# dalek-cryptography/curve25519-dalek

Hardware: NVIDIA H100
Metric: Pippenger MSM points/sec (higher is better)
Workload: dtype exact integers: f64 limbs (radix 2^51, FP64 pipe) in the bucket kernel, u32 limbs (radix 2^25.5) elsewhere

## Files before the change

curve25519_dalek_b200/csrc/api.cu:

```cuda
#include <cstring>
#include <new>
#include <random>

#include "../../include/dalek_b200.h"
#include "engine.h"

extern "C" {

int dalek_b200_init(int device, dalek_b200_ctx **out)
{
    if (!out) return DALEK_E_INVALID_ARG;
    *out = nullptr;
    int count = 0;
    if (cudaGetDeviceCount(&count) != cudaSuccess || count <= 0 || device < 0 || device >= count) return DALEK_E_NO_DEVICE;
    cudaDeviceProp prop;
    if (cudaGetDeviceProperties(&prop, device) != cudaSuccess) return DALEK_E_NO_DEVICE;
    if (prop.major != 9 || prop.minor != 0) return DALEK_E_NO_DEVICE;
    if (cudaSetDevice(device) != cudaSuccess) return DALEK_E_CUDA;
    dalek_b200_ctx *ctx = new (std::nothrow) dalek_b200_ctx();
    if (!ctx) return DALEK_E_NOMEM;
    ctx->device = device;
    ctx->sm_count = prop.multiProcessorCount;
    try { std::random_device rd; for (int i = 0; i < 4; i++) ctx->hash_seed[i] ^= rd(); } catch (...) { }
    int prio_lo = 0, prio_hi = 0;
    cudaDeviceGetStreamPriorityRange(&prio_lo, &prio_hi);
    if (cudaStreamCreateWithPriority(&ctx->stream, cudaStreamNonBlocking, prio_hi) != cudaSuccess ||
        cudaStreamCreateWithPriority(&ctx->stream2, cudaStreamNonBlocking, prio_lo) != cudaSuccess ||
        cudaStreamCreateWithFlags(&ctx->stream_copy, cudaStreamNonBlocking) != cudaSuccess ||
        cudaStreamCreateWithPriority(&ctx->stream3, cudaStreamNonBlocking, prio_hi) != cudaSuccess ||
        cudaStreamCreateWithPriority(&ctx->stream_hash, cudaStreamNonBlocking, prio_hi) != cudaSuccess ||
        cudaEventCreate(&ctx->ev_a) != cudaSuccess || cudaEventCreate(&ctx->ev_b) != cudaSuccess ||
        cudaEventCreate(&ctx->ev_call0) != cudaSuccess || cudaEventCreate(&ctx->ev_call1) != cudaSuccess ||
        cudaEventCreateWithFlags(&ctx->ev_fork, cudaEventDisableTiming) != cudaSuccess ||
        cudaEventCreateWithFlags(&ctx->ev_join, cudaEventDisableTiming) != cudaSuccess ||
        cudaEventCreateWithFlags(&ctx->ev_join2, cudaEventDisableTiming) != cudaSuccess) {
        delete ctx;
        return DALEK_E_CUDA;
    }
    for (int i = 0; i < 8; i++)
        if (cudaEventCreateWithFlags(&ctx->ev_grp[i], cudaEventDisableTiming) != cudaSuccess ||
            cudaEventCreateWithFlags(&ctx->ev_hram[i], cudaEventDisableTiming) != cudaSuccess || cudaEventCreate(&ctx->ev_prep[i][0]) != cudaSuccess ||
            cudaEventCreate(&ctx->ev_prep[i][1]) != cudaSuccess) { delete ctx; return DALEK_E_CUDA; }
    *out = ctx;
    return DALEK_OK;
}

void dalek_b200_destroy(dalek_b200_ctx *ctx)
{
    if (!ctx) return;
    cudaSetDevice(ctx->device);
    cudaStreamSynchronize(ctx->stream);
    cudaStreamSynchronize(ctx->stream2);
    cudaStreamSynchronize(ctx->stream3);
    cudaStreamSynchronize(ctx->stream_hash);
    DevBuf *bufs[] = {&ctx->scalars, &ctx->points_in, &ctx->points, &ctx->digits, &ctx->counts, &ctx->offsets,
                      &ctx->sorted, &ctx->buckets, &ctx->red_a, &ctx->red_b, &ctx->red_c, &ctx->red_d, &ctx->key_pts,
                      &ctx->result, &ctx->flags, &ctx->misc0, &ctx->misc1, &ctx->misc2, &ctx->misc3,
                      &ctx->misc4, &ctx->misc5, &ctx->zs, &ctx->base_table, &ctx->ntasks, &ctx->task_off, &ctx->tasks, &ctx->task_sums, &ctx->msg_offs, &ctx->sum_desc, &ctx->sum_part, &ctx->key_table, &ctx->key_acc, &ctx->task_order, &ctx->sig_status, &ctx->misc6, &ctx->each_pow, &ctx->each_tab, &ctx->each_kstat, &ctx->comb_base_table};
    for (DevBuf *b : bufs) if (b->p) cudaFree(b->p);
    if (ctx->h_pinned) cudaFreeHost(ctx->h_pinned);
    cudaEventDestroy(ctx->ev_a); cudaEventDestroy(ctx->ev_b); cudaEventDestroy(ctx->ev_fork); cudaEventDestroy(ctx->ev_join);
    cudaEventDestroy(ctx->ev_join2); cudaEventDestroy(ctx->ev_call0); cudaEventDestroy(ctx->ev_call1);
    for (int i = 0; i < 8; i++) { cudaEventDestroy(ctx->ev_grp[i]); cudaEventDestroy(ctx->ev_hram[i]); cudaEventDestroy(ctx->ev_prep[i][0]); cudaEventDestroy(ctx->ev_prep[i][1]); }
    cudaStreamDestroy(ctx->stream_hash);
    cudaStreamDestroy(ctx->stream); cudaStreamDestroy(ctx->stream2); cudaStreamDestroy(ctx->stream_copy); cudaStreamDestroy(ctx->stream3);
    delete ctx;
}

const char *dalek_b200_last_error(const dalek_b200_ctx *ctx) { return ctx ? ctx->last_error.c_str() : "null context"; }

int dalek_b200_set_option(dalek_b200_ctx *ctx, const char *name, long value)
{
    if (!ctx || !name) return DALEK_E_INVALID_ARG;
    if (!strcmp(name, "window_bits")) { if (value != 0 && (value < 4 || value > 20)) return DALEK_E_INVALID_ARG; ctx->opt_window_bits = value; return 0; }
    if (!strcmp(name, "host_chunks")) { if (value < 1 || value > 8) return DALEK_E_INVALID_ARG; ctx->opt_host_chunks = value; return 0; }
    if (!strcmp(name, "decompress_f64")) { ctx->opt_decompress_f64 = value ? 1 : 0; return 0; }
    if (!strcmp(name, "trace")) { ctx->opt_trace = value ? 1 : 0; return 0; }
    if (!strcmp(name, "precomp_tables")) { ctx->opt_precomp_tables = value ? 1 : 0; return 0; }
    if (!strcmp(name, "double_base_comb")) { ctx->opt_double_base_comb = value ? 1 : 0; return 0; }
    if (!strcmp(name, "dedupe_keys")) { ctx->opt_dedupe_keys = value ? 1 : 0; return 0; }
    if (!strcmp(name, "verify_pieces")) { if (value < 1 || value > 8) return DALEK_E_INVALID_ARG; ctx->opt_verify_pieces = value; return 0; }
    if (!strcmp(name, "transcript_warp")) { ctx->opt_transcript_warp = value ? 1 : 0; return 0; }
    if (!strcmp(name, "transcript_blocks")) { ctx->opt_transcript_blocks = value ? 1 : 0; return 0; }
    if (!strcmp(name, "each_comb")) { if (value < 0 || value > 2) return DALEK_E_INVALID_ARG; ctx->opt_each_comb = value; return 0; }
    if (!strcmp(name, "small_straus")) { ctx->opt_small_straus = value ? 1 : 0; return 0; }
    if (!strcmp(name, "acc_tma")) { ctx->opt_acc_tma = value ? 1 : 0; return 0; }
    if (!strcmp(name, "field_f64")) { ctx->opt_field_f64 = value ? 1 : 0; return 0; }
    if (!strcmp(name, "verify_chunk")) { if (value < 0 || value > (1 << 20)) return DALEK_E_INVALID_ARG; ctx->opt_verify_chunk = value; return 0; }
    return DALEK_E_INVALID_ARG;
}

uint64_t dalek_b200_launch_count(const dalek_b200_ctx *ctx) { return ctx ? ctx->launches : 0; }

int dalek_b200_last_kernel_ms(const dalek_b200_ctx *ctx, float *ms, int *launches)
{
    if (!ctx) return DALEK_E_INVALID_ARG;
    if (ms) *ms = ctx->last_kernel_ms;
    if (launches) *launches = ctx->last_kernel_launches;
    return 0;
}

int dalek_b200_last_stage_ms(const dalek_b200_ctx *ctx, const char *stage, float *ms)
{
    if (!ctx || !stage || !ms) return DALEK_E_INVALID_ARG;
    if (!strcmp(stage, "bucket_accumulate")) { *ms = ctx->last_kernel_ms; return 0; }
    if (!strcmp(stage, "decompress_R")) { *ms = ctx->last_prep_ms; return 0; }
    return DALEK_E_INVALID_ARG;
}

int dalek_b200_last_call_ms(const dalek_b200_ctx *ctx, float *ms)
{
    if (!ctx || !ms) return DALEK_E_INVALID_ARG;
    *ms = ctx->last_call_ms;
    return 0;
}

}

static int run_msm(dalek_b200_ctx *ctx, const void *scalars, const void *points_in, bool on_device, int point_fmt, size_t n,
                   size_t n_window ,
                   ge_p3_raw *d_windows, MsmResult *d_result)
{
    int rc;
    const size_t pin = msm_point_bytes(point_fmt);
    cudaStream_t st = ctx->stream;
    const int c = msm_choose_window_bits(ctx, n_window);
    const bool straus = d_result && n == n_window && n < STRAUS_VT_THRESHOLD && ctx->opt_small_straus && ctx->opt_field_f64;
    const int kind = msm_prepared_kind(point_fmt, straus ? PK_PNIELS : PK_NIELS);
    const size_t psz = kind == PK_NIELS ? sizeof(ge_niels_packed) : sizeof(ge_pniels_packed);
    if ((rc = ws_reserve(ctx, ctx->points, std::max<size_t>(1, n) * psz))) return rc;
    if ((rc = ws_reserve(ctx, ctx->flags, 64))) return rc;
    CUDA_TRY(ctx, cudaMemsetAsync(ctx->flags.p, 0, 64, st));
    if (on_device) {
        if (straus) {
            if ((rc = msm_prepare_points(ctx, points_in, point_fmt, n, ctx->points.p, (int *)ctx->flags.p, kind))) return rc;
            if ((rc = straus_vartime_msm(ctx, (const uint32_t *)scalars, ctx->points.p, kind, n, d_result))) return rc;
        } else {
            CUDA_TRY(ctx, cudaEventRecord(ctx->ev_fork, st));
            CUDA_TRY(ctx, cudaStreamWaitEvent(ctx->stream2, ctx->ev_fork, 0));
            if ((rc = msm_prepare_points_on(ctx, ctx->stream2, points_in, point_fmt, n, ctx->points.p, (int *)ctx->flags.p))) return rc;
            CUDA_TRY(ctx, cudaEventRecord(ctx->ev_join, ctx->stream2));
            if ((rc = msm_accumulate_chunk(ctx, (const uint32_t *)scalars, (const ge_niels_packed *)ctx->points.p, n, c, true, 0, 0, ctx->ev_join))) return rc;
        }
    } else {
        if ((rc = ws_reserve(ctx, ctx->scalars, std::max<size_t>(1, n) * 32))) return rc;
        if ((rc = ws_reserve(ctx, ctx->points_in, std::max<size_t>(1, n) * pin))) return rc;
        int K = n >= (1u << 18) ? (int)std::min<long>(8, std::max<long>(1, ctx->opt_host_chunks)) : 1;
        CUDA_TRY(ctx, cudaEventRecord(ctx->ev_fork, st));
        CUDA_TRY(ctx, cudaStreamWaitEvent(ctx->stream_copy, ctx->ev_fork, 0));
        CUDA_TRY(ctx, cudaStreamWaitEvent(ctx->stream2, ctx->ev_fork, 0));
        for (int k = 0; k < K; k++) {
            const size_t i0 = n * k / K, i1 = n * (k + 1) / K, cnt = i1 - i0;
            char *ds = (char *)ctx->scalars.p + i0 * 32, *dp = (char *)ctx->points_in.p + i0 * pin;
            if (cnt) {
                CUDA_TRY(ctx, cudaMemcpyAsync(ds, (const char *)scalars + i0 * 32, cnt * 32, cudaMemcpyHostToDevice, ctx->stream_copy));
                CUDA_TRY(ctx, cudaMemcpyAsync(dp, (const char *)points_in + i0 * pin, cnt * pin, cudaMemcpyHostToDevice, ctx->stream_copy));
            }
            CUDA_TRY(ctx, cudaEventRecord(ctx->ev_grp[k], ctx->stream_copy));
            CUDA_TRY(ctx, cudaStreamWaitEvent(st, ctx->ev_grp[k], 0));
            char *dq = (char *)ctx->points.p + i0 * psz;
            if (straus) {
                if ((rc = msm_prepare_points(ctx, dp, point_fmt, cnt, dq, (int *)ctx->flags.p, kind))) return rc;
                if ((rc = straus_vartime_msm(ctx, (const uint32_t *)ds, dq, kind, cnt, d_result))) return rc;
            } else {
                CUDA_TRY(ctx, cudaStreamWaitEvent(ctx->stream2, ctx->ev_grp[k], 0));
                if ((rc = msm_prepare_points_on(ctx, ctx->stream2, dp, point_fmt, cnt, dq, (int *)ctx->flags.p))) return rc;
                CUDA_TRY(ctx, cudaEventRecord(ctx->ev_join, ctx->stream2));
                if ((rc = msm_accumulate_chunk(ctx, (const uint32_t *)ds, (const ge_niels_packed *)dq, cnt, c, k == 0, 0, 0, ctx->ev_join))) return rc;
            }
        }
    }
    if (!straus && (rc = msm_reduce_finish(ctx, c, d_windows, d_result))) return rc;
    return 0;
}

int msm_read_result(dalek_b200_ctx *ctx, const MsmResult *d_result, const int *d_bad, const uint32_t *d_enc,
                    uint8_t out_compressed[32], uint64_t out_limbs[20])
{
    int rc;
    cudaStream_t st = ctx->stream;
    if ((rc = pinned_reserve(ctx, sizeof(MsmResult) + 128))) return rc;
    MsmResult *h = (MsmResult *)ctx->h_pinned;
    int *h_bad = (int *)((char *)ctx->h_pinned + sizeof(MsmResult));
    uint8_t *h_enc = (uint8_t *)ctx->h_pinned + sizeof(MsmResult) + 64;
    CUDA_TRY(ctx, cudaMemcpyAsync(h, d_result, sizeof(MsmResult), cudaMemcpyDeviceToHost, st));
    CUDA_TRY(ctx, cudaMemcpyAsync(h_bad, d_bad, sizeof(int), cudaMemcpyDeviceToHost, st));
    if (d_enc) CUDA_TRY(ctx, cudaMemcpyAsync(h_enc, d_enc, 32, cudaMemcpyDeviceToHost, st));
    CUDA_TRY(ctx, cudaStreamSynchronize(st));
    float ms = 0.f;
    if ((ms = elapsed_ms(ctx->ev_a, ctx->ev_b)) >= 0.f) ctx->last_kernel_ms = ms;
    if (out_compressed) memcpy(out_compressed, d_enc ? h_enc : (const uint8_t *)h->compressed, 32);
    if (out_limbs) memcpy(out_limbs, h->limbs, 160);
    return *h_bad ? DALEK_NONE : DALEK_OK;
}

static int msm_common(dalek_b200_ctx *ctx, const void *scalars, const void *points, bool on_device, int point_fmt,
                      size_t n, uint8_t out_compressed[32], uint64_t out_limbs[20])
{
    if (!ctx || (n && (!scalars || !points)) || n >= (1ull << 31)) return DALEK_E_INVALID_ARG;
    CUDA_TRY(ctx, cudaSetDevice(ctx->device));
    CallTimer timer(ctx);
    int rc;
    const int nwin = msm_window_count_for_bits(msm_choose_window_bits(ctx, n));
    if ((rc = ws_reserve(ctx, ctx->misc0, (size_t)nwin * sizeof(ge_p3_raw)))) return rc;
    if ((rc = ws_reserve(ctx, ctx->result, sizeof(MsmResult) + 32))) return rc;
    MsmResult *d_res = (MsmResult *)ctx->result.p;
    uint32_t *d_enc = point_fmt == DALEK_POINTS_RISTRETTO ? (uint32_t *)(d_res + 1) : nullptr;
    if ((rc = run_msm(ctx, scalars, points, on_device, point_fmt, n, n, (ge_p3_raw *)ctx->misc0.p, d_res))) return rc;
    if (d_enc && (rc = ristretto_encode_result(ctx, d_res, d_enc))) return rc;
    return msm_read_result(ctx, d_res, (const int *)ctx->flags.p, d_enc, out_compressed, out_limbs);
}
// ... 209 lines not shown
```

curve25519_dalek_b200/csrc/engine.h:

```cpp
#pragma once
#include <cuda_runtime.h>
#include <stddef.h>
#include <stdint.h>
#include <cstdio>
#include <string>
#include <utility>
#include <vector>

#include "../../include/dalek_b200.h"
#include "ge.cuh"

struct DevBuf {
    void *p = nullptr;
    size_t cap = 0;
};

struct dalek_b200_ctx {
    int device = 0;
    int sm_count = 132;
    cudaStream_t stream = nullptr;
    cudaStream_t stream2 = nullptr;
    cudaStream_t stream_copy = nullptr;
    cudaStream_t stream3 = nullptr;
    cudaStream_t stream_hash = nullptr;
    cudaEvent_t ev_hram[8] = {};
    cudaEvent_t ev_a = nullptr, ev_b = nullptr, ev_fork = nullptr, ev_join = nullptr, ev_join2 = nullptr;
    cudaEvent_t ev_call0 = nullptr, ev_call1 = nullptr;
    cudaEvent_t ev_prep[8][2] = {};
    int prep_pieces = 0;
    float last_prep_ms = 0.f;
    cudaEvent_t ev_grp[8] = {nullptr, nullptr, nullptr, nullptr, nullptr, nullptr, nullptr, nullptr};
    std::string last_error;
    uint64_t launches = 0;
    long opt_window_bits = 0;
    long opt_verify_chunk = 0;
    long opt_host_chunks = 8;
    long opt_trace = 0;
    long opt_precomp_tables = 0;
    long opt_double_base_comb = 1;
    long opt_dedupe_keys = 1;
    long opt_verify_pieces = 4;
    long opt_decompress_f64 = 1;
    long opt_acc_tma = 0;
    long opt_transcript_warp = 1;
    long opt_transcript_blocks = 1;
    long opt_each_comb = 1;
    long opt_small_straus = 1;
    long opt_field_f64 = 1;
    float last_kernel_ms = 0.f;
    float last_call_ms = 0.f;
    int last_kernel_launches = 0;
    bool async_open = false;
    DevBuf scalars, points_in, points, digits, counts, offsets, sorted, buckets, red_a, red_b, red_c,
        red_d, key_pts, result, flags, misc0, misc1, misc2, misc3, misc4, misc5, zs, base_table, ntasks, task_off, tasks, task_sums, msg_offs, sum_desc, sum_part, key_table, key_acc, task_order, sig_status, misc6, each_pow, each_tab, each_kstat;
    uint32_t hash_seed[4] = {0x243F6A88u, 0x85A308D3u, 0x13198A2Eu, 0x03707344u};
    int sum_desc_c = -1;
    bool base_table_ready = false;
    bool each_attr_set = false;
    bool comb_attr_set = false;
    DevBuf comb_base_table;
    bool comb_base_table_ready = false;
    void *h_pinned = nullptr;
    size_t h_pinned_cap = 0;
    size_t last_zs_n = 0;
    std::vector<std::pair<const char *, cudaEvent_t>> trace;
};

#define CUDA_TRY(ctx, expr)                                                                      \
    do {                                                                                         \
        cudaError_t _e = (expr);                                                                 \
        if (_e != cudaSuccess) {                                                                 \
            (ctx)->last_error = std::string(#expr) + ": " + cudaGetErrorString(_e);              \
            return -3;                                                                           \
        }                                                                                        \
    } while (0)

inline float elapsed_ms(cudaEvent_t a, cudaEvent_t b)
{
    float ms = 0.f;
    if (cudaEventElapsedTime(&ms, a, b) == cudaSuccess) return ms;
    cudaGetLastError();
    return -1.f;
}

struct CallTimer {
    dalek_b200_ctx *ctx;
    explicit CallTimer(dalek_b200_ctx *c) : ctx(c) { if (ctx) cudaEventRecord(ctx->ev_call0, ctx->stream); }
    ~CallTimer()
    {
        if (!ctx) return;
        float ms = 0.f;
        if (cudaEventRecord(ctx->ev_call1, ctx->stream) == cudaSuccess && cudaEventSynchronize(ctx->ev_call1) == cudaSuccess &&
            (ms = elapsed_ms(ctx->ev_call0, ctx->ev_call1)) >= 0.f)
            ctx->last_call_ms = ms;
    }
};

inline void trace_mark(dalek_b200_ctx *ctx, const char *name, cudaStream_t st)
{
    if (!ctx->opt_trace) return;
    cudaEvent_t e;
    if (cudaEventCreate(&e) != cudaSuccess) return;
    cudaEventRecord(e, st);
    ctx->trace.push_back({name, e});
}
inline void trace_dump(dalek_b200_ctx *ctx)
{
    if (!ctx->opt_trace) return;
    cudaDeviceSynchronize();
    for (auto &m : ctx->trace) {
        float ms = 0.f;
        cudaEventElapsedTime(&ms, ctx->ev_call0, m.second);
        fprintf(stderr, "[trace] %8.3f ms  %s\n", ms, m.first);
        cudaEventDestroy(m.second);
    }
    ctx->trace.clear();
}

inline bool flat_messages_ok(const uint8_t *msgs_flat, const uint64_t *offsets, size_t n)
{
    if (!n) return true;
    if (!offsets || offsets[0] != 0) return false;
    for (size_t i = 0; i < n; i++)
        if (offsets[i] > offsets[i + 1]) return false;
    return msgs_flat || offsets[n] == 0;
}

int ws_reserve(dalek_b200_ctx *ctx, DevBuf &b, size_t bytes);
int pinned_reserve(dalek_b200_ctx *ctx, size_t bytes);

enum { PK_NIELS = 0 , PK_PNIELS = 1  };

inline size_t msm_point_bytes(int point_fmt) { return point_fmt == DALEK_POINTS_EXTENDED ? 160 : 32; }

int msm_prepare_points(dalek_b200_ctx *ctx, const void *d_in, int point_fmt, size_t n, void *d_out,
                       int *d_bad, int kind = PK_NIELS);
int msm_prepared_kind(int point_fmt, int kind);

int msm_choose_window_bits(const dalek_b200_ctx *ctx, size_t n);
int msm_window_count_for_bits(int c);

struct MsmResult { uint32_t compressed[8]; uint64_t limbs[20]; uint32_t is_identity; uint32_t pad; };
int msm_accumulate_chunk(dalek_b200_ctx *ctx, const uint32_t *d_scalars, const ge_niels_packed *d_points, size_t n,
                         int c, bool first, int active_windows = 0, size_t flat = 0, cudaEvent_t points_ready = nullptr);
int msm_prepare_points_on(dalek_b200_ctx *ctx, cudaStream_t st, const void *d_in, int point_fmt, size_t n, void *d_out, int *d_bad,
                          int kind = PK_NIELS);
int msm_choose_window_bits_mixed(const dalek_b200_ctx *ctx, size_t n_short, int short_bits, size_t n_long);
int msm_reduce_finish(dalek_b200_ctx *ctx, int c, ge_p3_raw *d_windows, MsmResult *d_result, bool flat = false);
int msm_combine_windows(dalek_b200_ctx *ctx, const ge_p3_raw *d_windows, int ranks, int nwin, int c,
                        MsmResult *d_result);
int msm_read_result(dalek_b200_ctx *ctx, const MsmResult *d_result, const int *d_bad, const uint32_t *d_enc,
                    uint8_t out_compressed[32], uint64_t out_limbs[20]);

int msm_partial_enqueue_record(dalek_b200_ctx *ctx, const void *scalars, const void *points, bool on_device, int point_fmt,
                               size_t n_local, size_t n_shard, void *d_out_record, int dst_device);
int msm_combine_records(dalek_b200_ctx *ctx, const void *records, bool on_device, size_t rec_bytes, int ranks, size_t n_shard,
                        uint8_t out_compressed[32], uint64_t out_limbs[20]);

struct EachFront { const uint32_t *hs; const uint8_t *bad_s; const uint32_t *rep, *dense, *uniq; size_t nkeys; };
struct Sha512Prefix;
int verify_each_front(dalek_b200_ctx *ctx, const uint8_t *d_msgs, const uint64_t *d_offs, const uint32_t *d_sigs, const uint32_t *d_keys,
                      size_t n, EachFront *out, const Sha512Prefix *ph_dom = nullptr);

#define STRAUS_VT_THRESHOLD 190
int straus_vartime_msm(dalek_b200_ctx *ctx, const uint32_t *d_scalars, const void *d_points, int point_kind, size_t n,
                       MsmResult *d_result);

int straus_ct_msm(dalek_b200_ctx *ctx, const uint32_t *d_scalars, const void *d_points_pniels, size_t n,
                  MsmResult *d_result);
int base_table_ensure(dalek_b200_ctx *ctx);
#define COMB_BASE_DOUBLES (64 * 8 * 15)
int comb_base_table_ensure(dalek_b200_ctx *ctx);

int ristretto_encode_result(dalek_b200_ctx *ctx, const MsmResult *d_res, uint32_t *d_enc);
```

curve25519_dalek_b200/csrc/msm.cu:

```cuda
#include <algorithm>
#include <cstdio>
#include <utility>
#include <vector>

#include "../../include/dalek_b200.h"
#include "engine.h"
#include "ge64.cuh"
#include "warp4.cuh"
#include "warp4_f64.cuh"

static inline unsigned cdiv(size_t a, unsigned b) { return (unsigned)((a + b - 1) / b); }

int ws_reserve(dalek_b200_ctx *ctx, DevBuf &b, size_t bytes)
{
    if (bytes <= b.cap) return 0;
    if (b.p) { cudaFree(b.p); b.p = nullptr; b.cap = 0; }
    size_t want = bytes + bytes / 8 + 256;
    cudaError_t e = cudaMalloc(&b.p, want);
    if (e != cudaSuccess) { ctx->last_error = std::string("cudaMalloc: ") + cudaGetErrorString(e); return DALEK_E_NOMEM; }
    b.cap = want;
    return 0;
}

int pinned_reserve(dalek_b200_ctx *ctx, size_t bytes)
{
    if (bytes <= ctx->h_pinned_cap) return 0;
    if (ctx->h_pinned) cudaFreeHost(ctx->h_pinned);
    ctx->h_pinned = nullptr; ctx->h_pinned_cap = 0;
    cudaError_t e = cudaMallocHost(&ctx->h_pinned, bytes + 4096);
    if (e != cudaSuccess) { ctx->last_error = std::string("cudaMallocHost: ") + cudaGetErrorString(e); return DALEK_E_NOMEM; }
    ctx->h_pinned_cap = bytes + 4096;
    return 0;
}

template <int F64>
__global__ void __launch_bounds__(128, 3) k_prep_compressed(const uint4 *__restrict__ in, ge_niels_packed *__restrict__ out, size_t n,
                                  int *__restrict__ bad)
{
    size_t i = (size_t)blockIdx.x * blockDim.x + threadIdx.x;
    if (i >= n) return;
    uint4 a = in[2 * i], b = in[2 * i + 1];
    uint32_t s[8] = {a.x, a.y, a.z, a.w, b.x, b.y, b.z, b.w};
    fe x, y;
    uint32_t ok = ge_decompress_affine<F64>(x, y, s);
    if (!ok) { atomicOr(bad, 1); fe_0(x); fe_1(y); }
    ge_niels nl; ge_affine_to_niels(nl, x, y);
    ge_niels_packed p; ge_niels_pack(p, nl);
    uint4 *o = reinterpret_cast<uint4 *>(out + i);
#pragma unroll
    for (int k = 0; k < 6; k++) o[k] = make_uint4(p.w[4 * k], p.w[4 * k + 1], p.w[4 * k + 2], p.w[4 * k + 3]);
}

template <int F64>
__global__ void k_prep_ristretto(const uint32_t *__restrict__ in, ge_niels_packed *__restrict__ out, size_t n, int *__restrict__ bad)
{
    size_t i = (size_t)blockIdx.x * blockDim.x + threadIdx.x;
    if (i >= n) return;
    uint32_t enc[8];
#pragma unroll
    for (int k = 0; k < 8; k++) enc[k] = in[8 * i + k];
    ge_p3 P;
    if (!ristretto_decompress<F64>(P, enc)) { atomicOr(bad, 1); ge_p3_identity(P); }
    ge_niels nl; ge_affine_to_niels(nl, P.X, P.Y);
    ge_niels_packed pk; ge_niels_pack(pk, nl);
    out[i] = pk;
}

#define PREP_THREADS 128
#define PREP_PER_THREAD 8
#define PREP_GROUP (PREP_THREADS * PREP_PER_THREAD)

__device__ __forceinline__ void load_coord_f64(fe64 &h, const uint64_t *__restrict__ src)
{
    uint64_t l[5];
#pragma unroll
    for (int k = 0; k < 5; k++) l[k] = __ldg(src + k);
    fe t; fe_from_limbs51(t, l);
    fe64_from_fe_limbs(h, t);
}
__device__ __forceinline__ uint32_t fe64_nonzero(const fe64 &f)
{
    fe t; fe64_to_fe(t, f);
    return 1u - (uint32_t)fe_iszero(t);
}
__device__ __forceinline__ void fe64_shfl_up(fe64 &o, const fe64 &f, int d)
{
#pragma unroll
    for (int k = 0; k < 5; k++) o.v[k] = __shfl_up_sync(0xffffffffu, f.v[k], d);
}
__device__ __forceinline__ void fe64_shfl_down(fe64 &o, const fe64 &f, int d)
{
#pragma unroll
    for (int k = 0; k < 5; k++) o.v[k] = __shfl_down_sync(0xffffffffu, f.v[k], d);
}

__global__ void __launch_bounds__(PREP_THREADS, 3)
k_prep_extended(const uint64_t *__restrict__ in, ge_niels_packed *__restrict__ out, size_t n)
{
    constexpr int NW = PREP_THREADS / 32;
    __shared__ fe64 s_warp[NW];
    __shared__ fe64 s_pre[PREP_PER_THREAD][PREP_THREADS];
    const uint32_t tid = threadIdx.x, lane = tid & 31, warp = tid >> 5;
    const size_t g0 = (size_t)blockIdx.x * PREP_GROUP + tid;
    fe64 acc;
    uint32_t nz = 0;
    fe64_1(acc);
#pragma unroll 1
    for (int k = 0; k < PREP_PER_THREAD; k++) {
        const size_t i = g0 + (size_t)k * PREP_THREADS;
        if (i < n) {
            fe64 z, t;
            load_coord_f64(z, in + 20 * i + 10);
            const uint32_t ok = fe64_nonzero(z);
            fe64_mul(t, acc, z); fe64_cmov(acc, t, ok);
            nz |= ok << k;
        }
        s_pre[k][tid] = acc;
    }
    fe64 lo = acc, hi = acc, t;
#pragma unroll 1
    for (int d = 1; d < 32; d <<= 1) {
        fe64_shfl_up(t, lo, d);
        if (lane >= (uint32_t)d) fe64_mul(lo, lo, t);
        fe64_shfl_down(t, hi, d);
        if (lane + d < 32) fe64_mul(hi, hi, t);
    }
    if (lane == 31) s_warp[warp] = lo;
    fe64_shfl_up(t, lo, 1); lo = t; if (lane == 0) fe64_1(lo);
    fe64_shfl_down(t, hi, 1); hi = t; if (lane == 31) fe64_1(hi);
    __syncthreads();
    if (tid == 0) {
        fe64 run[NW], inv;
        run[0] = s_warp[0];
#pragma unroll
        for (int w = 1; w < NW; w++) fe64_mul(run[w], run[w - 1], s_warp[w]);
        {
            fe q; fe64_to_fe(q, run[NW - 1]); fe_invert(q, q); fe64_from_fe_limbs(inv, q);
        }
#pragma unroll
        for (int w = NW - 1; w > 0; w--) {
            fe64 iw;
            fe64_mul(iw, inv, run[w - 1]);
            fe64_mul(inv, inv, s_warp[w]);
            s_warp[w] = iw;
        }
        s_warp[0] = inv;
    }
    __syncthreads();
    fe64 inv;
    fe64_mul(inv, s_warp[warp], lo); fe64_mul(inv, inv, hi);
#pragma unroll 1
    for (int k = PREP_PER_THREAD - 1; k >= 0; k--) {
        const size_t i = g0 + (size_t)k * PREP_THREADS;
        if (i >= n) continue;
        const uint32_t ok = (nz >> k) & 1u;
        const uint64_t *src = in + 20 * i;
        fe64 X, Y, zi, u, v;
        load_coord_f64(u, src + 10);
        if (k > 0) fe64_mul(zi, inv, s_pre[k - 1][tid]); else zi = inv;
        fe64_mul(v, inv, u); fe64_cmov(inv, v, ok);
        ge_niels_packed pk;
        fe f;
        load_coord_f64(X, src); load_coord_f64(Y, src + 5);
        fe64_add(u, Y, X); fe64_mul(v, u, zi);
        fe64_to_fe(f, v); fe_tobytes_words(pk.w, f);
        fe64_sub(u, Y, X); fe64_mul(v, u, zi);
        fe64_to_fe(f, v); fe_tobytes_words(pk.w + 8, f);
        load_coord_f64(u, src + 15);
        fe64_mul(v, u, zi); fe64_const_2d(u); fe64_mul(v, v, u);
        fe64_to_fe(f, v); fe_tobytes_words(pk.w + 16, f);
#pragma unroll
        for (int q = 0; q < 24; q++) pk.w[q] = ok ? pk.w[q] : (q == 0 || q == 8 ? 1u : 0u);
        uint4 *o = reinterpret_cast<uint4 *>(out + i);
#pragma unroll
        for (int q = 0; q < 6; q++) o[q] = make_uint4(pk.w[4 * q], pk.w[4 * q + 1], pk.w[4 * q + 2], pk.w[4 * q + 3]);
    }
}

__global__ void k_prep_extended_pniels(const uint64_t *__restrict__ in, ge_pniels_packed *__restrict__ out, size_t n)
{
    size_t i = (size_t)blockIdx.x * blockDim.x + threadIdx.x;
    if (i >= n) return;
    const ulonglong2 *src = reinterpret_cast<const ulonglong2 *>(in + 20 * i);
    uint64_t l[20];
#pragma unroll
    for (int k = 0; k < 10; k++) { ulonglong2 v = src[k]; l[2 * k] = v.x; l[2 * k + 1] = v.y; }
    ge_p3 p;
    fe_from_limbs51(p.X, l); fe_from_limbs51(p.Y, l + 5); fe_from_limbs51(p.Z, l + 10); fe_from_limbs51(p.T, l + 15);
    ge_pniels pn; ge_p3_to_pniels(pn, p);
    ge_pniels_packed pk; ge_pniels_pack(pk, pn);
    uint4 *o = reinterpret_cast<uint4 *>(out + i);
#pragma unroll
    for (int k = 0; k < 8; k++) o[k] = make_uint4(pk.w[4 * k], pk.w[4 * k + 1], pk.w[4 * k + 2], pk.w[4 * k + 3]);
}

int msm_prepared_kind(int point_fmt, int kind)
{
    return point_fmt == DALEK_POINTS_EXTENDED ? kind : PK_NIELS;
}

int msm_prepare_points_on(dalek_b200_ctx *ctx, cudaStream_t st, const void *d_in, int point_fmt, size_t n, void *d_out, int *d_bad,
                          int kind)
{
    if (n == 0) return 0;
    if (point_fmt == DALEK_POINTS_COMPRESSED) {
        if (ctx->opt_decompress_f64) k_prep_compressed<1><<<cdiv(n, 128), 128, 0, st>>>((const uint4 *)d_in, (ge_niels_packed *)d_out, n, d_bad);
        else k_prep_compressed<0><<<cdiv(n, 128), 128, 0, st>>>((const uint4 *)d_in, (ge_niels_packed *)d_out, n, d_bad);
    } else if (point_fmt == DALEK_POINTS_RISTRETTO) {
        if (ctx->opt_decompress_f64) k_prep_ristretto<1><<<cdiv(n, 128), 128, 0, st>>>((const uint32_t *)d_in, (ge_niels_packed *)d_out, n, d_bad);
        else k_prep_ristretto<0><<<cdiv(n, 128), 128, 0, st>>>((const uint32_t *)d_in, (ge_niels_packed *)d_out, n, d_bad);
    } else if (kind == PK_PNIELS) {
        k_prep_extended_pniels<<<cdiv(n, 128), 128, 0, st>>>((const uint64_t *)d_in, (ge_pniels_packed *)d_out, n);
    } else {
        k_prep_extended<<<cdiv(n, PREP_GROUP), PREP_THREADS, 0, st>>>((const uint64_t *)d_in, (ge_niels_packed *)d_out, n);
    }
    ctx->launches++;
    CUDA_TRY(ctx, cudaGetLastError());
    return 0;
}

int msm_prepare_points(dalek_b200_ctx *ctx, const void *d_in, int point_fmt, size_t n, void *d_out, int *d_bad, int kind)
{
    return msm_prepare_points_on(ctx, ctx->stream, d_in, point_fmt, n, d_out, d_bad, kind);
}

int msm_window_count_for_bits(int c) { return 256 / c + 1; }

int msm_choose_window_bits(const dalek_b200_ctx *ctx, size_t n)
{
    if (ctx->opt_window_bits >= 4 && ctx->opt_window_bits <= 20) return (int)ctx->opt_window_bits;
    int best = 4; double best_cost = 1e300;
    for (int c = 4; c <= 20; c++) {
        double W = (double)((253 + c - 1) / c);
        double cost = W * ((double)n + 4.0 * (double)(1u << (c - 1)));
        if (cost < best_cost) { best_cost = cost; best = c; }
    }
    return best;
}

int msm_choose_window_bits_mixed(const dalek_b200_ctx *ctx, size_t n_short, int short_bits, size_t n_long)
{
    if (ctx->opt_window_bits >= 4 && ctx->opt_window_bits <= 20) return (int)ctx->opt_window_bits;
    int best = 4; double best_cost = 1e300;
    for (int c = 4; c <= 20; c++) {
        double W = (double)((253 + c - 1) / c), Ws = (double)((short_bits + 1 + c - 1) / c);
        double cost = Ws * (double)n_short + W * ((double)n_long + 4.0 * (double)(1u << (c - 1)));
        if (cost < best_cost) { best_cost = cost; best = c; }
    }
    return best;
}

#define SORT_THREADS 512
#define SORT_COUNT_TILE 4096u
#define SORT_TILE 2048u
#define SORT_HIST_MAX 8192u
#define SORT_NC_MAX 4096u
#define SORT_FINE_MAX 12
#define SORT_BIN_MEAN 4096u
#define SORT_FINE_CAP 8192u

__device__ __forceinline__ int32_t next_digit(uint32_t s[8], uint32_t &carry, int c)
{
    const uint32_t v = (s[0] & ((1u << c) - 1)) + carry;
#pragma unroll
    for (int k = 0; k < 7; k++) s[k] = __funnelshift_r(s[k], s[k + 1], c);
    s[7] >>= c;
    if (v > (1u << (c - 1))) { carry = 1; return (int32_t)v - (int32_t)(1u << c); }
    carry = 0;
    return (int32_t)v;
}

__device__ __forceinline__ void load_scalar(uint32_t s[8], const uint4 *__restrict__ scalars, size_t i)
{
    const uint4 a = scalars[2 * i], b = scalars[2 * i + 1];
    s[0] = a.x; s[1] = a.y; s[2] = a.z; s[3] = a.w; s[4] = b.x; s[5] = b.y; s[6] = b.z; s[7] = b.w;
}

__device__ uint32_t block_excl_scan(uint32_t *v, uint32_t len, uint32_t *scr)
{
    const uint32_t t = threadIdx.x, lane = t & 31, wid = t >> 5, nw = blockDim.x >> 5;
    const uint32_t per = (len + blockDim.x - 1) / blockDim.x, b = min(t * per, len), e = min(b + per, len);
    __syncthreads();
    uint32_t sum = 0;
    for (uint32_t k = b; k < e; k++) sum += v[k];
    uint32_t incl = sum;
    for (int d = 1; d < 32; d <<= 1) { uint32_t x = __shfl_up_sync(0xffffffffu, incl, d); if (lane >= (uint32_t)d) incl += x; }
    if (lane == 31) scr[wid] = incl;
    __syncthreads();
    if (wid == 0) {
        const uint32_t x = lane < nw ? scr[lane] : 0;
        uint32_t y = x;
        for (int d = 1; d < 32; d <<= 1) { uint32_t z = __shfl_up_sync(0xffffffffu, y, d); if (lane >= (uint32_t)d) y += z; }
        if (lane < nw) scr[lane] = y - x;
        if (lane == 31) scr[32] = y;
    }
    __syncthreads();
    uint32_t run = scr[wid] + incl - sum;
    for (uint32_t k = b; k < e; k++) { const uint32_t x = v[k]; v[k] = run; run += x; }
    const uint32_t total = scr[32];
    __syncthreads();
    return total;
}

__device__ __forceinline__ uint32_t warp_claim(uint32_t *ctr, uint32_t key, bool live)
{
    const uint32_t lane = threadIdx.x & 31;
    const uint32_t peers = __match_any_sync(0xffffffffu, live ? key : 0xffffffffu);
    const uint32_t leader = __ffs(peers) - 1;
    uint32_t base = 0;
    if (live && lane == leader) base = atomicAdd(&ctr[key], (uint32_t)__popc(peers));
    base = __shfl_sync(0xffffffffu, base, leader);
    return base + __popc(peers & ((1u << lane) - 1));
}

__global__ void __launch_bounds__(SORT_THREADS)
k_sort_count(const uint4 *__restrict__ scalars, size_t n, int c, int nact, int F, uint32_t nc, int flat,
             uint32_t *__restrict__ ccount)
{
    __shared__ uint32_t h[SORT_HIST_MAX];
    const uint32_t nh = (flat ? 1u : (uint32_t)nact) * nc;
    for (uint32_t k = threadIdx.x; k < nh; k += SORT_THREADS) h[k] = 0;
    __syncthreads();
    for (uint32_t j = 0; j < SORT_COUNT_TILE / SORT_THREADS; j++) {
        const size_t i = (size_t)blockIdx.x * SORT_COUNT_TILE + j * SORT_THREADS + threadIdx.x;
        if (i >= n) break;
        uint32_t s[8], carry = 0;
        load_scalar(s, scalars, i);
        for (int w = 0; w < nact; w++) {
            const int32_t d = next_digit(s, carry, c);
            if (d) atomicAdd(&h[(flat ? 0u : (uint32_t)w * nc) + (((uint32_t)(d < 0 ? -d : d) - 1) >> F)], 1u);
        }
    }
    __syncthreads();
    for (uint32_t k = threadIdx.x; k < nh; k += SORT_THREADS)
        if (h[k]) atomicAdd(&ccount[k], h[k]);
}

__device__ __forceinline__ uint32_t extra_slices(uint32_t cnt) { return cnt > SORT_FINE_CAP ? (cnt - 1) / SORT_FINE_CAP : 0; }

__global__ void __launch_bounds__(SORT_THREADS)
k_sort_bins_scan(const uint32_t *__restrict__ ccount, uint32_t nc, int F, uint32_t nbuckets, uint32_t *__restrict__ ccursor,
                 uint32_t *__restrict__ xpre, uint32_t *__restrict__ xtot, uint32_t *__restrict__ counts,
                 uint32_t *__restrict__ fill)
{
    __shared__ uint32_t v[SORT_NC_MAX], scr[33];
    const size_t o = (size_t)blockIdx.x * nc;
    for (uint32_t k = threadIdx.x; k < nc; k += SORT_THREADS) v[k] = ccount[o + k];
    block_excl_scan(v, nc, scr);
    for (uint32_t k = threadIdx.x; k < nc; k += SORT_THREADS) { ccursor[o + k] = v[k]; v[k] = extra_slices(ccount[o + k]); }
    const uint32_t total = block_excl_scan(v, nc, scr);
    for (uint32_t k = threadIdx.x; k < nc; k += SORT_THREADS) xpre[o + k] = v[k];
    if (threadIdx.x == 0) xtot[blockIdx.x] = total;
    for (uint32_t k = 0; k < nc; k++) {
        if ((k + 1 < nc ? v[k + 1] : total) == v[k]) continue;
        const size_t b0 = (size_t)blockIdx.x * nbuckets + ((size_t)k << F);
        for (uint32_t f = threadIdx.x; f < (1u << F); f += SORT_THREADS) { counts[b0 + f] = 0; fill[b0 + f] = 0; }
    }
}

__global__ void __launch_bounds__(SORT_THREADS, 2)
k_sort_partition(const uint4 *__restrict__ scalars, size_t n, int c, int nact, int F, uint32_t nc, uint32_t nbuckets, size_t flat,
                 const uint32_t *__restrict__ ccount, uint32_t *__restrict__ ccursor, uint2 *__restrict__ records,
                 uint32_t *__restrict__ counts)
{
    constexpr int SPT = SORT_TILE / SORT_THREADS;
    extern __shared__ uint32_t sm[];
    uint2 *stage = reinterpret_cast<uint2 *>(sm);
// ... 764 lines not shown
```

Before: 328.7 million.

## Share one field inversion across all blocks in extended-point preparation

```diff
diff --git a/curve25519_dalek_b200/csrc/api.cu b/curve25519_dalek_b200/csrc/api.cu
--- a/curve25519_dalek_b200/csrc/api.cu
+++ b/curve25519_dalek_b200/csrc/api.cu
@@ -56,7 +56,7 @@
     DevBuf *bufs[] = {&ctx->scalars, &ctx->points_in, &ctx->points, &ctx->digits, &ctx->counts, &ctx->offsets,
                       &ctx->sorted, &ctx->buckets, &ctx->red_a, &ctx->red_b, &ctx->red_c, &ctx->red_d, &ctx->key_pts,
                       &ctx->result, &ctx->flags, &ctx->misc0, &ctx->misc1, &ctx->misc2, &ctx->misc3,
-                      &ctx->misc4, &ctx->misc5, &ctx->zs, &ctx->base_table, &ctx->ntasks, &ctx->task_off, &ctx->tasks, &ctx->task_sums, &ctx->msg_offs, &ctx->sum_desc, &ctx->sum_part, &ctx->key_table, &ctx->key_acc, &ctx->task_order, &ctx->sig_status, &ctx->misc6, &ctx->each_pow, &ctx->each_tab, &ctx->each_kstat, &ctx->comb_base_table};
+                      &ctx->misc4, &ctx->misc5, &ctx->zs, &ctx->base_table, &ctx->ntasks, &ctx->task_off, &ctx->tasks, &ctx->task_sums, &ctx->msg_offs, &ctx->sum_desc, &ctx->sum_part, &ctx->key_table, &ctx->key_acc, &ctx->task_order, &ctx->sig_status, &ctx->misc6, &ctx->each_pow, &ctx->each_tab, &ctx->each_kstat, &ctx->comb_base_table, &ctx->prep_prod};
     for (DevBuf *b : bufs) if (b->p) cudaFree(b->p);
     if (ctx->h_pinned) cudaFreeHost(ctx->h_pinned);
     cudaEventDestroy(ctx->ev_a); cudaEventDestroy(ctx->ev_b); cudaEventDestroy(ctx->ev_fork); cudaEventDestroy(ctx->ev_join);
diff --git a/curve25519_dalek_b200/csrc/engine.h b/curve25519_dalek_b200/csrc/engine.h
--- a/curve25519_dalek_b200/csrc/engine.h
+++ b/curve25519_dalek_b200/csrc/engine.h
@@ -53,6 +53,7 @@
     bool async_open = false;
     DevBuf scalars, points_in, points, digits, counts, offsets, sorted, buckets, red_a, red_b, red_c,
         red_d, key_pts, result, flags, misc0, misc1, misc2, misc3, misc4, misc5, zs, base_table, ntasks, task_off, tasks, task_sums, msg_offs, sum_desc, sum_part, key_table, key_acc, task_order, sig_status, misc6, each_pow, each_tab, each_kstat;
+    DevBuf prep_prod;
     uint32_t hash_seed[4] = {0x243F6A88u, 0x85A308D3u, 0x13198A2Eu, 0x03707344u};
     int sum_desc_c = -1;
     bool base_table_ready = false;
diff --git a/curve25519_dalek_b200/csrc/msm.cu b/curve25519_dalek_b200/csrc/msm.cu
--- a/curve25519_dalek_b200/csrc/msm.cu
+++ b/curve25519_dalek_b200/csrc/msm.cu
@@ -66,9 +66,10 @@
     out[i] = pk;
 }
 
-#define PREP_THREADS 128
-#define PREP_PER_THREAD 8
+#define PREP_THREADS 256
+#define PREP_PER_THREAD 4
 #define PREP_GROUP (PREP_THREADS * PREP_PER_THREAD)
+#define PREP_NW (PREP_THREADS / 32)
 
 __device__ __forceinline__ void load_coord_f64(fe64 &h, const uint64_t *__restrict__ src)
 {
@@ -78,9 +79,23 @@
     fe t; fe_from_limbs51(t, l);
     fe64_from_fe_limbs(h, t);
 }
-__device__ __forceinline__ uint32_t fe64_nonzero(const fe64 &f)
-{
-    fe t; fe64_to_fe(t, f);
+__device__ __forceinline__ void store_coord(uint4 *o, const fe64 &v, uint32_t ok, uint32_t c)
+{
+    fe f;
+    uint32_t w[8];
+    fe64_to_fe(f, v); fe_tobytes_words(w, f);
+#pragma unroll
+    for (int q = 0; q < 8; q++) w[q] = ok ? w[q] : (q == 0 ? c : 0u);
+    o[0] = make_uint4(w[0], w[1], w[2], w[3]);
+    o[1] = make_uint4(w[4], w[5], w[6], w[7]);
+}
+__device__ __forceinline__ uint32_t load_z(fe64 &h, const uint64_t *__restrict__ in, size_t i)
+{
+    uint64_t l[5];
+#pragma unroll
+    for (int k = 0; k < 5; k++) l[k] = __ldg(in + 20 * i + 10 + k);
+    fe t; fe_from_limbs51(t, l);
+    fe64_from_fe_limbs(h, t);
     return 1u - (uint32_t)fe_iszero(t);
 }
 __device__ __forceinline__ void fe64_shfl_up(fe64 &o, const fe64 &f, int d)
@@ -93,31 +108,29 @@
 #pragma unroll
     for (int k = 0; k < 5; k++) o.v[k] = __shfl_down_sync(0xffffffffu, f.v[k], d);
 }
-
-__global__ void __launch_bounds__(PREP_THREADS, 3)
-k_prep_extended(const uint64_t *__restrict__ in, ge_niels_packed *__restrict__ out, size_t n)
-{
-    constexpr int NW = PREP_THREADS / 32;
-    __shared__ fe64 s_warp[NW];
-    __shared__ fe64 s_pre[PREP_PER_THREAD][PREP_THREADS];
-    const uint32_t tid = threadIdx.x, lane = tid & 31, warp = tid >> 5;
-    const size_t g0 = (size_t)blockIdx.x * PREP_GROUP + tid;
-    fe64 acc;
-    uint32_t nz = 0;
-    fe64_1(acc);
+__device__ __forceinline__ void fe64_shfl_xor(fe64 &o, const fe64 &f, int m)
+{
+#pragma unroll
+    for (int k = 0; k < 5; k++) o.v[k] = __shfl_xor_sync(0xffffffffu, f.v[k], m);
+}
+__device__ __forceinline__ void fe64_shfl_idx(fe64 &o, const fe64 &f, int src)
+{
+#pragma unroll
+    for (int k = 0; k < 5; k++) o.v[k] = __shfl_sync(0xffffffffu, f.v[k], src);
+}
+
+__device__ __forceinline__ void warp_product(fe64 &p, const fe64 &x, int width)
+{
+    fe64 t;
+    p = x;
 #pragma unroll 1
-    for (int k = 0; k < PREP_PER_THREAD; k++) {
-        const size_t i = g0 + (size_t)k * PREP_THREADS;
-        if (i < n) {
-            fe64 z, t;
-            load_coord_f64(z, in + 20 * i + 10);
-            const uint32_t ok = fe64_nonzero(z);
-            fe64_mul(t, acc, z); fe64_cmov(acc, t, ok);
-            nz |= ok << k;
-        }
-        s_pre[k][tid] = acc;
-    }
-    fe64 lo = acc, hi = acc, t;
+    for (int m = width >> 1; m > 0; m >>= 1) { fe64_shfl_xor(t, p, m); fe64_mul(p, p, t); }
+}
+
+__device__ __forceinline__ void warp_other_products(const fe64 &x, fe64 &below, fe64 &above, fe64 &all)
+{
+    const uint32_t lane = threadIdx.x & 31;
+    fe64 lo = x, hi = x, t;
 #pragma unroll 1
     for (int d = 1; d < 32; d <<= 1) {
         fe64_shfl_up(t, lo, d);
@@ -125,30 +138,101 @@
         fe64_shfl_down(t, hi, d);
         if (lane + d < 32) fe64_mul(hi, hi, t);
     }
-    if (lane == 31) s_warp[warp] = lo;
-    fe64_shfl_up(t, lo, 1); lo = t; if (lane == 0) fe64_1(lo);
-    fe64_shfl_down(t, hi, 1); hi = t; if (lane == 31) fe64_1(hi);
-    __syncthreads();
-    if (tid == 0) {
-        fe64 run[NW], inv;
-        run[0] = s_warp[0];
-#pragma unroll
-        for (int w = 1; w < NW; w++) fe64_mul(run[w], run[w - 1], s_warp[w]);
-        {
-            fe q; fe64_to_fe(q, run[NW - 1]); fe_invert(q, q); fe64_from_fe_limbs(inv, q);
-        }
-#pragma unroll
-        for (int w = NW - 1; w > 0; w--) {
-            fe64 iw;
-            fe64_mul(iw, inv, run[w - 1]);
-            fe64_mul(inv, inv, s_warp[w]);
-            s_warp[w] = iw;
-        }
-        s_warp[0] = inv;
-    }
-    __syncthreads();
-    fe64 inv;
-    fe64_mul(inv, s_warp[warp], lo); fe64_mul(inv, inv, hi);
+    fe64_shfl_idx(all, lo, 31);
+    fe64_shfl_up(below, lo, 1); if (lane == 0) fe64_1(below);
+    fe64_shfl_down(above, hi, 1); if (lane == 31) fe64_1(above);
+}
+
+template <bool INVERT>
+__device__ __forceinline__ void block_inverse(fe64 &inv, const fe64 &acc, fe64 *s_warp, const fe64 *tot_inv)
+{
+    const uint32_t lane = threadIdx.x & 31, warp = threadIdx.x >> 5, nw = blockDim.x >> 5;
+    fe64 below, above, all;
+    warp_other_products(acc, below, above, all);
+    if (lane == 0) s_warp[warp] = all;
+    __syncthreads();
+    if (warp == 0) {
+        fe64 x, b, a, t;
+        if (lane < nw) x = s_warp[lane]; else fe64_1(x);
+        warp_other_products(x, b, a, all);
+        if (INVERT) {
+            fe q; fe64_to_fe(q, all); fe_invert(q, q); fe64_from_fe_limbs(t, q);
+        } else {
+            t = *tot_inv;
+        }
+        fe64_mul(t, t, b); fe64_mul(t, t, a);
+        if (lane < nw) s_warp[lane] = t;
+    }
+    __syncthreads();
+    fe64_mul(inv, s_warp[warp], below); fe64_mul(inv, inv, above);
+}
+
+__global__ void __launch_bounds__(PREP_THREADS, 2)
+k_prep_zprod(const uint64_t *__restrict__ in, fe64 *__restrict__ prod, size_t n)
+{
+    __shared__ fe64 s_warp[PREP_NW];
+    const uint32_t tid = threadIdx.x, lane = tid & 31, warp = tid >> 5;
+    const size_t g0 = (size_t)blockIdx.x * PREP_GROUP + tid;
+    fe64 z[PREP_PER_THREAD], acc, t;
+    uint32_t ok[PREP_PER_THREAD];
+#pragma unroll
+    for (int k = 0; k < PREP_PER_THREAD; k++) {
+        const size_t i = g0 + (size_t)k * PREP_THREADS;
+        if (i < n) ok[k] = load_z(z[k], in, i); else { ok[k] = 0; fe64_1(z[k]); }
+    }
+    acc = z[0];
+    if (!ok[0]) fe64_1(acc);
+#pragma unroll
+    for (int k = 1; k < PREP_PER_THREAD; k++) { fe64_mul(t, acc, z[k]); fe64_cmov(acc, t, ok[k]); }
+    warp_product(t, acc, 32);
+    if (lane == 0) s_warp[warp] = t;
+    __syncthreads();
+    if (warp == 0) {
+        if (lane < PREP_NW) acc = s_warp[lane]; else fe64_1(acc);
+        warp_product(t, acc, PREP_NW);
+        if (lane == 0) prod[blockIdx.x] = t;
+    }
+}
+
+__global__ void __launch_bounds__(PREP_THREADS)
+k_prep_invert(fe64 *__restrict__ prod, fe64 *__restrict__ pre, uint32_t G)
+{
+    __shared__ fe64 s_warp[PREP_NW];
+    const uint32_t per = (G + blockDim.x - 1) / blockDim.x, b = min(threadIdx.x * per, G), e = min(b + per, G);
+    fe64 acc, inv, t;
+    fe64_1(acc);
+    for (uint32_t k = b; k < e; k++) { fe64_mul(acc, acc, prod[k]); pre[k] = acc; }
+    block_inverse<true>(inv, acc, s_warp, nullptr);
+    for (uint32_t k = e; k-- > b;) {
+        const fe64 x = prod[k];
+        if (k > b) fe64_mul(t, inv, pre[k - 1]); else t = inv;
+        prod[k] = t;
+        fe64_mul(inv, inv, x);
+    }
+}
+
+__global__ void __launch_bounds__(PREP_THREADS, 2)
+k_prep_finish(const uint64_t *__restrict__ in, const fe64 *__restrict__ ginv, ge_niels_packed *__restrict__ out, size_t n)
+{
+    __shared__ fe64 s_warp[PREP_NW];
+    __shared__ fe64 s_pre[PREP_PER_THREAD - 1][PREP_THREADS];
+    const uint32_t tid = threadIdx.x;
+    const size_t g0 = (size_t)blockIdx.x * PREP_GROUP + tid;
+    fe64 acc, inv;
+    uint32_t nz = 0;
+    fe64_1(acc);
+#pragma unroll 1
+    for (int k = 0; k < PREP_PER_THREAD; k++) {
+        const size_t i = g0 + (size_t)k * PREP_THREADS;
+        if (k > 0) s_pre[k - 1][tid] = acc;
+        if (i < n) {
+            fe64 z, t;
+            const uint32_t ok = load_z(z, in, i);
+            fe64_mul(t, acc, z); fe64_cmov(acc, t, ok);
+            nz |= ok << k;
+        }
+    }
+    block_inverse<false>(inv, acc, s_warp, ginv + blockIdx.x);
 #pragma unroll 1
     for (int k = PREP_PER_THREAD - 1; k >= 0; k--) {
         const size_t i = g0 + (size_t)k * PREP_THREADS;
@@ -159,21 +243,15 @@
         load_coord_f64(u, src + 10);
         if (k > 0) fe64_mul(zi, inv, s_pre[k - 1][tid]); else zi = inv;
         fe64_mul(v, inv, u); fe64_cmov(inv, v, ok);
-        ge_niels_packed pk;
-        fe f;
+        uint4 *o = reinterpret_cast<uint4 *>(out + i);
         load_coord_f64(X, src); load_coord_f64(Y, src + 5);
         fe64_add(u, Y, X); fe64_mul(v, u, zi);
-        fe64_to_fe(f, v); fe_tobytes_words(pk.w, f);
+        store_coord(o, v, ok, 1u);
         fe64_sub(u, Y, X); fe64_mul(v, u, zi);
-        fe64_to_fe(f, v); fe_tobytes_words(pk.w + 8, f);
+        store_coord(o + 2, v, ok, 1u);
         load_coord_f64(u, src + 15);
         fe64_mul(v, u, zi); fe64_const_2d(u); fe64_mul(v, v, u);
-        fe64_to_fe(f, v); fe_tobytes_words(pk.w + 16, f);
-#pragma unroll
-        for (int q = 0; q < 24; q++) pk.w[q] = ok ? pk.w[q] : (q == 0 || q == 8 ? 1u : 0u);
-        uint4 *o = reinterpret_cast<uint4 *>(out + i);
-#pragma unroll
-        for (int q = 0; q < 6; q++) o[q] = make_uint4(pk.w[4 * q], pk.w[4 * q + 1], pk.w[4 * q + 2], pk.w[4 * q + 3]);
+        store_coord(o + 4, v, ok, 0u);
     }
 }
 
@@ -212,7 +290,14 @@
     } else if (kind == PK_PNIELS) {
         k_prep_extended_pniels<<<cdiv(n, 128), 128, 0, st>>>((const uint64_t *)d_in, (ge_pniels_packed *)d_out, n);
     } else {
-        k_prep_extended<<<cdiv(n, PREP_GROUP), PREP_THREADS, 0, st>>>((const uint64_t *)d_in, (ge_niels_packed *)d_out, n);
+        const unsigned G = cdiv(n, PREP_GROUP);
+        int rc;
+        if ((rc = ws_reserve(ctx, ctx->prep_prod, 2 * (size_t)G * sizeof(fe64)))) return rc;
+        fe64 *prod = (fe64 *)ctx->prep_prod.p;
+        k_prep_zprod<<<G, PREP_THREADS, 0, st>>>((const uint64_t *)d_in, prod, n);
+        k_prep_invert<<<1, PREP_THREADS, 0, st>>>(prod, prod + G, G);
+        k_prep_finish<<<G, PREP_THREADS, 0, st>>>((const uint64_t *)d_in, prod, (ge_niels_packed *)d_out, n);
+        ctx->launches += 2;
     }
     ctx->launches++;
     CUDA_TRY(ctx, cudaGetLastError());
```

New measurement: 358.7 million, median of 6. +9.1%, better.
